# szlbiubiubiu/LAFS_CVPR2024

Measured on AMD Instinct MI355X. Metric: face-crops/sec/node (ViT-S LAFS pretrain, 2g+8l crops), higher is better.
Workload: dtype bf16; 1 GPU; vit_small/8 LAFS pretrain step, 2 global 112x112 + 8 local 48x48 crops, batch 64/GPU, out_dim 100000, drop_path 0.1, dp1; global_batch=64, parallelism=dp1, hip_graph=True, landmark_frontend_in_step=False, device_augmentation_in_step=False

## Files before the change

lafs_cvpr2024_amd/csrc/gemm_kres.hip:

```cpp
#include <stdlib.h>
#include "common.hpp"
#include "gemm_plan.hpp"
#include "ctx.hpp"

namespace {

typedef unsigned int u32x4_t __attribute__((ext_vector_type(4)));
typedef float f32x4v_t __attribute__((ext_vector_type(4)));

constexpr int KK = 384;
constexpr int CPR = KK / 8;
constexpr int ROWB = KK * 2;
constexpr int GROWS = 32;
constexpr int STAGE = GROWS * ROWB;
constexpr int NSTG = 3;
constexpr int NTH = 256;
constexpr int NDMA4 = STAGE / 16 / NTH;
constexpr int NKK = KK / 32;
constexpr int MAXN = 1536;
constexpr int FD = 8;
static_assert(CPR % 16 == 0 && STAGE % (16 * NTH) == 0, "stage layout");

struct KArgs {
  const bf16_t* A; const bf16_t* B;
  int M, N, lda, ldb;
  void* C; int ldc; void* C2; int ldc2;
  const float* bias; const float* resid; int ldr;
  const float* seq_scale; const int* row2seq;
  const bf16_t* aux; int ldaux;
  int cbn, items;
  int save_grad;
};

template <int N> __device__ __forceinline__ void wait_vm() { asm volatile("s_waitcnt vmcnt(%0)" ::"n"(N) : "memory"); }
__device__ __forceinline__ void fence() { asm volatile("" ::: "memory"); }
__device__ __forceinline__ void st16(void* p, unsigned a, unsigned b, unsigned c, unsigned d) {
  const u32x4_t v = {a, b, c, d};
  *reinterpret_cast<u32x4_t*>(p) = v;
}
__device__ __forceinline__ void st16f(void* p, float a, float b, float c, float d) {
  const f32x4v_t v = {a, b, c, d};
  *reinterpret_cast<f32x4v_t*>(p) = v;
}

template <int EPI, bool HAS_U> struct EpiOps {
  static constexpr bool F32 = (EPI == LAFS_EPI_RESID_F32);
  static constexpr int S = F32 ? 8 : ((EPI == LAFS_EPI_BF16_GELU && HAS_U) ? 8 : 4);
  static constexpr int P = F32 ? 8 : ((EPI == LAFS_EPI_DGELU_BF16) ? 4 : 0);
};

template <int EPI, bool HAS_U>
__global__ __launch_bounds__(NTH, 2) void gemm_kres_kernel(KArgs p) {
  constexpr int UROWS = 128, NDMA = NDMA4;
  constexpr int S = EpiOps<EPI, HAS_U>::S, P = EpiOps<EPI, HAS_U>::P;
  constexpr bool F32 = EpiOps<EPI, HAS_U>::F32;
  constexpr bool AUX_IS_GRAD = (EPI == LAFS_EPI_DGELU_BF16) && !HAS_U;
  __shared__ __attribute__((aligned(16))) unsigned char smem[NSTG * STAGE];
  __shared__ __attribute__((aligned(16))) float sbias[MAXN];
  const int tid = threadIdx.x, lane = tid & 63;
  const int wave = __builtin_amdgcn_readfirstlane(tid >> 6);
  const int t = lane & 15, q = lane >> 4;
  const int G = (int)gridDim.x, per = G >> 3;
  const int id = (blockIdx.x & 7) * per + (blockIdx.x >> 3);
  const int ib = (int)((long)p.items * id / G), ie = (int)((long)p.items * (id + 1) / G);
  if (ie <= ib) return;

  for (int i = tid; i < p.N; i += NTH) sbias[i] = p.bias ? p.bias[i] : 0.f;
  __syncthreads();

  int doff[NDMA];
#pragma unroll
  for (int i = 0; i < NDMA; ++i) {
    const int x = i * NTH + tid, rho = x / CPR, cp = x % CPR, c = cp ^ (rho & 15);
    const int s16 = rho & 15, gi = rho >> 4;
    const int rowrel = F32 ? rho : (8 * (s16 >> 2) + 4 * gi + (s16 & 3));
    doff[i] = (rowrel * p.ldb + c * 8) * 2;
  }
  const int cbn = p.cbn;
  const unsigned lds0 = lds_addr_of(smem);
  int pstage = 0;
  auto issue = [&](int k) {
    const int cb = (k >> 1) % cbn;
    const bf16_t* base = p.B + (size_t)(cb * 64 + 32 * (k & 1)) * p.ldb;
    const unsigned st = lds0 + pstage * STAGE + wave * 1024;
    pstage = (pstage + 1 == NSTG) ? 0 : pstage + 1;
    fence();
#pragma unroll
    for (int i = 0; i < NDMA; ++i) lds_dma16_m0_s(base, (unsigned)doff[i], st + i * (NTH * 16));
    fence();
  };
  auto issue_rows = [&](int mu, int w, int buf) {
    const unsigned st = lds0 + buf * STAGE + wave * 1024;
    fence();
#pragma unroll
    for (int i = 0; i < NDMA; ++i) {
      const int x = i * NTH + tid, rho = x / CPR, cp = x % CPR, c = cp ^ (rho & 15);
      const int row = min(mu * UROWS + w * 32 + rho, p.M - 1);
      lds_dma16_m0(p.A + (size_t)row * p.lda + c * 8, st + i * (NTH * 16));
    }
    fence();
  };

  int foff[4];
#pragma unroll
  for (int i = 0; i < 4; ++i) {
    foff[i] = t * ROWB + (((4 * i + q) ^ t) << 4);
    asm volatile("" : "+v"(foff[i]));
  }
  bf16x8_t areg[2][NKK];
  f32x4_t acc[2][2][2];
  uint4 pre[P > 0 ? P : 1];
  float sc[2] = {1.0f, 1.0f};
  int cur_mu = -1;
  bool active = false;
  int m0 = 0;

  auto fetch = [&](int item, uint4 (&dst)[P > 0 ? P : 1]) {
    if (P == 0) return;
    const int it = min(item, p.items - 1);
    const int mu = it / cbn, n0 = (it - mu * cbn) * 64;
#pragma unroll
    for (int i = 0; i < P; ++i) {
      const int b = i & 1, x = i >> 1;
      const int mr = min(mu * UROWS + wave * 32 + t + 16 * b, p.M - 1);
      if (F32) dst[i] = *reinterpret_cast<const uint4*>(p.resid + (size_t)mr * p.ldr + n0 + 16 * x + 4 * q);
      else dst[i] = *reinterpret_cast<const uint4*>(p.aux + (size_t)mr * p.ldaux + n0 + 32 * x + 8 * q);
    }
    fence();
  };
  auto bias_init = [&](f32x4_t (&a)[2][2], int n0, int g) {
#pragma unroll
    for (int gi = 0; gi < 2; ++gi) {
      const int n = F32 ? n0 + 16 * (2 * g + gi) + 4 * q : n0 + 32 * g + 8 * q + 4 * gi;
#pragma unroll
      for (int b = 0; b < 2; ++b) a[gi][b] = *reinterpret_cast<const f32x4_t*>(sbias + n);
    }
  };
  auto mfma_stage = [&](int stage, f32x4_t (&a)[2][2]) {
    __builtin_amdgcn_sched_barrier(0);
    const unsigned char* st = smem + stage * STAGE;
#pragma unroll
    for (int kk = 0; kk < NKK; ++kk)
#pragma unroll
      for (int gi = 0; gi < 2; ++gi) {
        const bf16x8_t w = *reinterpret_cast<const bf16x8_t*>(st + foff[kk & 3] + (kk >> 2) * 256 + gi * (16 * ROWB));
        a[gi][0] = mfma16(w, areg[0][kk], a[gi][0]);
        a[gi][1] = mfma16(w, areg[1][kk], a[gi][1]);
      }
    __builtin_amdgcn_sched_group_barrier(0x100, FD, 0);
#pragma unroll
    for (int i = 0; i < 2 * NKK - FD; ++i) {
      __builtin_amdgcn_sched_group_barrier(0x008, 2, 0);
      __builtin_amdgcn_sched_group_barrier(0x100, 1, 0);
    }
    __builtin_amdgcn_sched_group_barrier(0x008, 2 * FD, 0);
    __builtin_amdgcn_sched_barrier(0);
  };

  auto read_rows = [&](int buf) {
    const unsigned char* st = smem + buf * STAGE;
#pragma unroll
    for (int b = 0; b < 2; ++b)
#pragma unroll
      for (int kk = 0; kk < NKK; ++kk)
        areg[b][kk] = *reinterpret_cast<const bf16x8_t*>(st + foff[kk & 3] + (kk >> 2) * 256 + b * (16 * ROWB));
    asm volatile("s_waitcnt lgkmcnt(0)" ::: "memory");
  };
  int stage = 0;
  bool fresh = false;
  for (int it = ib; it < ie; ++it) {
    const int mu = it / cbn, cb = it - mu * cbn;
    const int k0 = 2 * it;
    const bool feed_next = (it + 1 < ie) && ((it + 1) / cbn == mu);
    bias_init(acc[0], cb * 64, 0);
    if (mu != cur_mu) {
      cur_mu = mu;
      m0 = mu * UROWS + wave * 32 + t;
      active = (mu * UROWS + wave * 32) < p.M;
      if (EPI == LAFS_EPI_RESID_F32 && p.seq_scale != nullptr) {
#pragma unroll
        for (int b = 0; b < 2; ++b) sc[b] = p.seq_scale[p.row2seq[min(m0 + 16 * b, p.M - 1)]];
      }
      wait_vm<0>();
      __builtin_amdgcn_s_barrier();
      issue_rows(mu, 0, 0); issue_rows(mu, 1, 1); issue_rows(mu, 2, 2);
      wait_vm<0>();
      __builtin_amdgcn_s_barrier();
      if (wave < 3) read_rows(wave);
      __builtin_amdgcn_s_barrier();
      issue_rows(mu, 3, 0);
      pstage = 1;
      issue(k0);
      issue(k0 + 1);
      wait_vm<2 * NDMA>();
      __builtin_amdgcn_s_barrier();
      if (wave == 3) read_rows(0);
      stage = 1;
      wait_vm<NDMA>();
      fresh = true;
    } else {
      if (active) wait_vm<NDMA + S + P>(); else wait_vm<NDMA + P>();
    }
    __builtin_amdgcn_s_barrier();
    if (feed_next) issue(k0 + 2);
    bias_init(acc[1], cb * 64, 1);
    mfma_stage(stage, acc[0]);
    stage = (stage + 1 == NSTG) ? 0 : stage + 1;
    if (fresh) {
      if (feed_next) wait_vm<NDMA>(); else wait_vm<0>();
    } else if (feed_next) {
      if (active) wait_vm<NDMA + S + P>(); else wait_vm<NDMA + P>();
    } else {
      if (active) wait_vm<S + P>(); else wait_vm<P>();
    }
    fresh = false;
    __builtin_amdgcn_s_barrier();
    if (feed_next) issue(k0 + 3);
    fetch(it, pre);
    mfma_stage(stage, acc[1]);
    stage = (stage + 1 == NSTG) ? 0 : stage + 1;

    fence();
    const int n0 = cb * 64;
    if (active) {
#pragma unroll
      for (int b = 0; b < 2; ++b) {
        const int m = m0 + 16 * b;
        const bool rowok = (m < p.M);
        if (F32) {
#pragma unroll
          for (int x = 0; x < 4; ++x) {
            const int g = x >> 1, gi = x & 1;
            const int n = n0 + 16 * x + 4 * q;
            const uint4 r4 = pre[x * 2 + b];
            float v0 = acc[g][gi][b][0], v1 = acc[g][gi][b][1], v2 = acc[g][gi][b][2], v3 = acc[g][gi][b][3];
            v0 = __uint_as_float(r4.x) + sc[b] * v0; v1 = __uint_as_float(r4.y) + sc[b] * v1;
            v2 = __uint_as_float(r4.z) + sc[b] * v2; v3 = __uint_as_float(r4.w) + sc[b] * v3;
            if (rowok) st16f(reinterpret_cast<float*>(p.C) + (size_t)m * p.ldc + n, v0, v1, v2, v3);
          }
        } else {
          float v[2][8];
#pragma unroll
          for (int g = 0; g < 2; ++g) {
            v[g][0] = acc[g][0][b][0]; v[g][1] = acc[g][0][b][1]; v[g][2] = acc[g][0][b][2]; v[g][3] = acc[g][0][b][3];
            v[g][4] = acc[g][1][b][0]; v[g][5] = acc[g][1][b][1]; v[g][6] = acc[g][1][b][2]; v[g][7] = acc[g][1][b][3];
            if (EPI == LAFS_EPI_DGELU_BF16) {
              const uint4 a4 = pre[g * 2 + b];
              if constexpr (AUX_IS_GRAD) {
                v[g][0] *= bf_lo(a4.x); v[g][1] *= bf_hi(a4.x); v[g][2] *= bf_lo(a4.y); v[g][3] *= bf_hi(a4.y);
                v[g][4] *= bf_lo(a4.z); v[g][5] *= bf_hi(a4.z); v[g][6] *= bf_lo(a4.w); v[g][7] *= bf_hi(a4.w);
              } else {
                v[g][0] *= gelu_grad_f(bf_lo(a4.x)); v[g][1] *= gelu_grad_f(bf_hi(a4.x)); v[g][2] *= gelu_grad_f(bf_lo(a4.y)); v[g][3] *= gelu_grad_f(bf_hi(a4.y));
                v[g][4] *= gelu_grad_f(bf_lo(a4.z)); v[g][5] *= gelu_grad_f(bf_hi(a4.z)); v[g][6] *= gelu_grad_f(bf_lo(a4.w)); v[g][7] *= gelu_grad_f(bf_hi(a4.w));
              }
            }
          }
          float dv[2][8];
          const bool both = (EPI == LAFS_EPI_BF16_GELU) && HAS_U && p.save_grad;
          if (both) {
#pragma unroll
            for (int g = 0; g < 2; ++g)
#pragma unroll
              for (int e = 0; e < 8; ++e) { float gv; gelu_both_f(v[g][e], gv, dv[g][e]); v[g][e] = gv; }
#pragma unroll
            for (int g = 0; g < 2; ++g) {
              const int n = n0 + 32 * g + 8 * q;
              if (rowok) st16(reinterpret_cast<bf16_t*>(p.C) + (size_t)m * p.ldc + n, pack_bf2(dv[g][0], dv[g][1]), pack_bf2(dv[g][2], dv[g][3]),
                              pack_bf2(dv[g][4], dv[g][5]), pack_bf2(dv[g][6], dv[g][7]));
            }
          }
          if ((EPI != LAFS_EPI_BF16_GELU || HAS_U) && !both) {
#pragma unroll
            for (int g = 0; g < 2; ++g) {
              const int n = n0 + 32 * g + 8 * q;
              if (rowok) st16(reinterpret_cast<bf16_t*>(p.C) + (size_t)m * p.ldc + n, pack_bf2(v[g][0], v[g][1]), pack_bf2(v[g][2], v[g][3]),
                              pack_bf2(v[g][4], v[g][5]), pack_bf2(v[g][6], v[g][7]));
            }
          }
          if (EPI == LAFS_EPI_BF16_GELU) {
            if (!both) {
#pragma unroll
              for (int g = 0; g < 2; ++g)
#pragma unroll
                for (int e = 0; e < 8; ++e) v[g][e] = gelu_f(v[g][e]);
            }
#pragma unroll
            for (int g = 0; g < 2; ++g) {
              const int n = n0 + 32 * g + 8 * q;
              if (rowok) st16(reinterpret_cast<bf16_t*>(p.C2) + (size_t)m * p.ldc2 + n, pack_bf2(v[g][0], v[g][1]), pack_bf2(v[g][2], v[g][3]),
                              pack_bf2(v[g][4], v[g][5]), pack_bf2(v[g][6], v[g][7]));
            }
          }
        }
      }
    }
    fence();
  }
}

template <int EPI, bool HAS_U>
int launch(const KArgs& a, int grid, hipStream_t s) {
  hipLaunchKernelGGL((gemm_kres_kernel<EPI, HAS_U>), dim3(grid), dim3(NTH), 0, s, a);
  LAFS_LAUNCH_CHECK();
  return LAFS_OK;
}

}

bool lafs_kres_eligible(const lafs_gemm_nt_args* g, NtPlan* p) {
  const int mask = lafs_ctx_opt(g->ctx, LAFS_OPT_KRES_MASK);
  const int e = g->epilogue;
  const int bit = e == LAFS_EPI_BF16 ? 1 : (e == LAFS_EPI_BF16_GELU ? 2 : (e == LAFS_EPI_RESID_F32 ? 4 : (e == LAFS_EPI_DGELU_BF16 ? 8 : 0)));
  if (!(mask & bit)) return false;
  if (g->splits > 1 || g->operand_f16) return false;
  if (g->K != KK || g->N % 64 != 0 || g->N > MAXN || g->N < 64 || g->M < 2048) return false;
  if (g->drop_p > 0.f) return false;
  if (g->C == nullptr && g->ldc % 8 != 0) return false;
  const int items = ((g->M + 127) / 128) * (g->N / 64);
  const int min_items = lafs_ctx_opt(g->ctx, LAFS_OPT_KRES_MIN_ITEMS);
  const int g_comm_cus = lafs_ctx_opt(g->ctx, LAFS_OPT_COMM_CUS);
  int grid = 512;
  while (grid > 8 && items / grid < min_items) grid >>= 1;
  if (g_comm_cus > 0 && grid > 2 * (256 - g_comm_cus)) grid = (2 * (256 - g_comm_cus)) & ~7;
  p->info = { 1,  128,  64,  KK,  NTH,  0,  1,  grid};
  return true;
}

int lafs_kres_launch(const lafs_gemm_nt_args* g, const NtPlan& p, hipStream_t stream) {
  const int e = g->epilogue;
  KArgs a;
  a.A = (const bf16_t*)g->A; a.B = (const bf16_t*)g->B; a.M = g->M; a.N = g->N; a.lda = g->lda; a.ldb = g->ldb;
  a.C = g->C; a.ldc = g->ldc; a.C2 = g->C2; a.ldc2 = g->ldc2;
  a.bias = (e == LAFS_EPI_DGELU_BF16) ? nullptr : g->bias;
  a.resid = g->resid; a.ldr = g->ldr; a.seq_scale = g->seq_scale; a.row2seq = g->row2seq;
  a.aux = (const bf16_t*)g->aux; a.ldaux = g->ldaux;
  a.cbn = g->N / 64;
  a.save_grad = (g->act == LAFS_GELU_SAVE_GRAD && (e == LAFS_EPI_BF16_GELU || e == LAFS_EPI_DGELU_BF16)) ? 1 : 0;
  a.items = ((g->M + 127) / 128) * a.cbn;
  const int grid = p.info.workgroups;
  switch (e) {
    case LAFS_EPI_BF16: return launch<LAFS_EPI_BF16, true>(a, grid, stream);
    case LAFS_EPI_BF16_GELU:
      return g->C != nullptr ? launch<LAFS_EPI_BF16_GELU, true>(a, grid, stream) : launch<LAFS_EPI_BF16_GELU, false>(a, grid, stream);
    case LAFS_EPI_RESID_F32: return launch<LAFS_EPI_RESID_F32, true>(a, grid, stream);
    default:
      return a.save_grad ? launch<LAFS_EPI_DGELU_BF16, false>(a, grid, stream) : launch<LAFS_EPI_DGELU_BF16, true>(a, grid, stream);
  }
}
```

lafs_cvpr2024_amd/csrc/gemm_plan.hpp:

```cpp
#pragma once
#include "lafs_hip.h"

struct NtPlan {
  lafs_gemm_nt_plan_info info;
  int inst, klen;
  int geo;
};

bool lafs_kres_eligible(const lafs_gemm_nt_args* g, NtPlan* p);
int lafs_kres_launch(const lafs_gemm_nt_args* g, const NtPlan& p, hipStream_t stream);
bool lafs_big_eligible(const lafs_gemm_nt_args* g, NtPlan* p);
int lafs_big_launch(const lafs_gemm_nt_args* g, const NtPlan& p, hipStream_t stream);
```

Baseline: 45550 face-crops/s.

## Partition K-resident GEMM work by row-unit aligned column splits

Replaces the flat linear split of (row-unit, column-block) items across workgroups with a partition where each workgroup owns one 128-row unit and a contiguous slice of its column blocks, when that balances well enough. The restructured loop nests column blocks inside row units, so each workgroup loads its A rows exactly once and avoids row reloads at item-range boundaries. Bias loading now overlaps with the initial row DMA, and the min-items grid-shrinking knob is dropped. This can change the grid size and load balance, and it falls back to the linear split when the partition would be too uneven.

```diff
diff --git a/lafs_cvpr2024_amd/csrc/gemm_kres.hip b/lafs_cvpr2024_amd/csrc/gemm_kres.hip
--- a/lafs_cvpr2024_amd/csrc/gemm_kres.hip
+++ b/lafs_cvpr2024_amd/csrc/gemm_kres.hip
@@ -28,9 +28,18 @@
   const float* bias; const float* resid; int ldr;
   const float* seq_scale; const int* row2seq;
   const bf16_t* aux; int ldaux;
-  int cbn, items;
+  int cbn, units, parts;
   int save_grad;
 };
+
+struct KresGrid { int parts, grid; };
+inline KresGrid kres_partition(int units, int cbn, int slots) {
+  int parts = slots / units;
+  parts = parts > cbn ? cbn : parts;
+  const long items = (long)units * cbn;
+  if (parts < 1 || 2L * ((cbn + parts - 1) / parts) * slots > 2 * items + 3L * slots) return {0, slots};
+  return {parts, (units * parts + 7) & ~7};
+}
 
 template <int N> __device__ __forceinline__ void wait_vm() { asm volatile("s_waitcnt vmcnt(%0)" ::"n"(N) : "memory"); }
 __device__ __forceinline__ void fence() { asm volatile("" ::: "memory"); }
@@ -62,11 +71,19 @@
   const int t = lane & 15, q = lane >> 4;
   const int G = (int)gridDim.x, per = G >> 3;
   const int id = (blockIdx.x & 7) * per + (blockIdx.x >> 3);
-  const int ib = (int)((long)p.items * id / G), ie = (int)((long)p.items * (id + 1) / G);
-  if (ie <= ib) return;
-
-  for (int i = tid; i < p.N; i += NTH) sbias[i] = p.bias ? p.bias[i] : 0.f;
-  __syncthreads();
+  const int cbn = p.cbn;
+  int ib, ie;
+  if (p.parts > 0) {
+    const int part = id % p.parts, unit = id / p.parts;
+    if (unit >= p.units) return;
+    ib = unit * cbn + cbn * part / p.parts;
+    ie = unit * cbn + cbn * (part + 1) / p.parts;
+  } else {
+    const long items = (long)p.units * cbn;
+    ib = (int)(items * id / G);
+    ie = (int)(items * (id + 1) / G);
+    if (ie <= ib) return;
+  }
 
   int doff[NDMA];
 #pragma unroll
@@ -76,12 +93,10 @@
     const int rowrel = F32 ? rho : (8 * (s16 >> 2) + 4 * gi + (s16 & 3));
     doff[i] = (rowrel * p.ldb + c * 8) * 2;
   }
-  const int cbn = p.cbn;
   const unsigned lds0 = lds_addr_of(smem);
   int pstage = 0;
   auto issue = [&](int k) {
-    const int cb = (k >> 1) % cbn;
-    const bf16_t* base = p.B + (size_t)(cb * 64 + 32 * (k & 1)) * p.ldb;
+    const bf16_t* base = p.B + (size_t)(32 * k) * p.ldb;
     const unsigned st = lds0 + pstage * STAGE + wave * 1024;
     pstage = (pstage + 1 == NSTG) ? 0 : pstage + 1;
     fence();
@@ -111,18 +126,16 @@
   f32x4_t acc[2][2][2];
   uint4 pre[P > 0 ? P : 1];
   float sc[2] = {1.0f, 1.0f};
-  int cur_mu = -1;
   bool active = false;
   int m0 = 0;
 
-  auto fetch = [&](int item, uint4 (&dst)[P > 0 ? P : 1]) {
+  auto fetch = [&](int cb, uint4 (&dst)[P > 0 ? P : 1]) {
     if (P == 0) return;
-    const int it = min(item, p.items - 1);
-    const int mu = it / cbn, n0 = (it - mu * cbn) * 64;
+    const int n0 = cb * 64;
 #pragma unroll
     for (int i = 0; i < P; ++i) {
       const int b = i & 1, x = i >> 1;
-      const int mr = min(mu * UROWS + wave * 32 + t + 16 * b, p.M - 1);
+      const int mr = min(m0 + 16 * b, p.M - 1);
       if (F32) dst[i] = *reinterpret_cast<const uint4*>(p.resid + (size_t)mr * p.ldr + n0 + 16 * x + 4 * q);
       else dst[i] = *reinterpret_cast<const uint4*>(p.aux + (size_t)mr * p.ldaux + n0 + 32 * x + 8 * q);
     }
@@ -166,135 +179,134 @@
         areg[b][kk] = *reinterpret_cast<const bf16x8_t*>(st + foff[kk & 3] + (kk >> 2) * 256 + b * (16 * ROWB));
     asm volatile("s_waitcnt lgkmcnt(0)" ::: "memory");
   };
-  int stage = 0;
-  bool fresh = false;
-  for (int it = ib; it < ie; ++it) {
-    const int mu = it / cbn, cb = it - mu * cbn;
-    const int k0 = 2 * it;
-    const bool feed_next = (it + 1 < ie) && ((it + 1) / cbn == mu);
-    bias_init(acc[0], cb * 64, 0);
-    if (mu != cur_mu) {
-      cur_mu = mu;
-      m0 = mu * UROWS + wave * 32 + t;
-      active = (mu * UROWS + wave * 32) < p.M;
-      if (EPI == LAFS_EPI_RESID_F32 && p.seq_scale != nullptr) {
-#pragma unroll
-        for (int b = 0; b < 2; ++b) sc[b] = p.seq_scale[p.row2seq[min(m0 + 16 * b, p.M - 1)]];
+  const int mu0 = ib / cbn;
+  for (int mu = mu0; mu * cbn < ie; ++mu) {
+    const bool first_unit = (mu == mu0);
+    const int cb0 = max(ib - mu * cbn, 0), cb1 = min(ie - mu * cbn, cbn);
+    m0 = mu * UROWS + wave * 32 + t;
+    active = (mu * UROWS + wave * 32) < p.M;
+    if (!first_unit) __builtin_amdgcn_s_barrier();
+    issue_rows(mu, 0, 0); issue_rows(mu, 1, 1); issue_rows(mu, 2, 2);
+    if (first_unit)
+      for (int i = tid; i < p.N; i += NTH) sbias[i] = p.bias ? p.bias[i] : 0.f;
+    if (EPI == LAFS_EPI_RESID_F32 && p.seq_scale != nullptr) {
+#pragma unroll
+      for (int b = 0; b < 2; ++b) sc[b] = p.seq_scale[p.row2seq[min(m0 + 16 * b, p.M - 1)]];
+    }
+    wait_vm<0>();
+    __syncthreads();
+    if (wave < 3) read_rows(wave);
+    __builtin_amdgcn_s_barrier();
+    issue_rows(mu, 3, 0);
+    pstage = 1;
+    issue(2 * cb0);
+    issue(2 * cb0 + 1);
+    wait_vm<2 * NDMA>();
+    __builtin_amdgcn_s_barrier();
+    if (wave == 3) read_rows(0);
+    int stage = 1;
+    for (int cb = cb0; cb < cb1; ++cb) {
+      const int k0 = 2 * cb;
+      const bool first = (cb == cb0);
+      const bool feed_next = (cb + 1 < cb1);
+      bias_init(acc[0], cb * 64, 0);
+      if (first) wait_vm<NDMA>();
+      else if (active) wait_vm<NDMA + S + P>();
+      else wait_vm<NDMA + P>();
+      __builtin_amdgcn_s_barrier();
+      if (feed_next) issue(k0 + 2);
+      bias_init(acc[1], cb * 64, 1);
+      mfma_stage(stage, acc[0]);
+      stage = (stage + 1 == NSTG) ? 0 : stage + 1;
+      if (first) {
+        if (feed_next) wait_vm<NDMA>(); else wait_vm<0>();
+      } else if (feed_next) {
+        if (active) wait_vm<NDMA + S + P>(); else wait_vm<NDMA + P>();
+      } else {
+        if (active) wait_vm<S + P>(); else wait_vm<P>();
       }
-      wait_vm<0>();
       __builtin_amdgcn_s_barrier();
-      issue_rows(mu, 0, 0); issue_rows(mu, 1, 1); issue_rows(mu, 2, 2);
-      wait_vm<0>();
-      __builtin_amdgcn_s_barrier();
-      if (wave < 3) read_rows(wave);
-      __builtin_amdgcn_s_barrier();
-      issue_rows(mu, 3, 0);
-      pstage = 1;
-      issue(k0);
-      issue(k0 + 1);
-      wait_vm<2 * NDMA>();
-      __builtin_amdgcn_s_barrier();
-      if (wave == 3) read_rows(0);
-      stage = 1;
-      wait_vm<NDMA>();
-      fresh = true;
-    } else {
-      if (active) wait_vm<NDMA + S + P>(); else wait_vm<NDMA + P>();
-    }
-    __builtin_amdgcn_s_barrier();
-    if (feed_next) issue(k0 + 2);
-    bias_init(acc[1], cb * 64, 1);
-    mfma_stage(stage, acc[0]);
-    stage = (stage + 1 == NSTG) ? 0 : stage + 1;
-    if (fresh) {
-      if (feed_next) wait_vm<NDMA>(); else wait_vm<0>();
-    } else if (feed_next) {
-      if (active) wait_vm<NDMA + S + P>(); else wait_vm<NDMA + P>();
-    } else {
-      if (active) wait_vm<S + P>(); else wait_vm<P>();
-    }
-    fresh = false;
-    __builtin_amdgcn_s_barrier();
-    if (feed_next) issue(k0 + 3);
-    fetch(it, pre);
-    mfma_stage(stage, acc[1]);
-    stage = (stage + 1 == NSTG) ? 0 : stage + 1;
-
-    fence();
-    const int n0 = cb * 64;
-    if (active) {
-#pragma unroll
-      for (int b = 0; b < 2; ++b) {
-        const int m = m0 + 16 * b;
-        const bool rowok = (m < p.M);
-        if (F32) {
-#pragma unroll
-          for (int x = 0; x < 4; ++x) {
-            const int g = x >> 1, gi = x & 1;
-            const int n = n0 + 16 * x + 4 * q;
-            const uint4 r4 = pre[x * 2 + b];
-            float v0 = acc[g][gi][b][0], v1 = acc[g][gi][b][1], v2 = acc[g][gi][b][2], v3 = acc[g][gi][b][3];
-            v0 = __uint_as_float(r4.x) + sc[b] * v0; v1 = __uint_as_float(r4.y) + sc[b] * v1;
-            v2 = __uint_as_float(r4.z) + sc[b] * v2; v3 = __uint_as_float(r4.w) + sc[b] * v3;
-            if (rowok) st16f(reinterpret_cast<float*>(p.C) + (size_t)m * p.ldc + n, v0, v1, v2, v3);
-          }
-        } else {
-          float v[2][8];
-#pragma unroll
-          for (int g = 0; g < 2; ++g) {
-            v[g][0] = acc[g][0][b][0]; v[g][1] = acc[g][0][b][1]; v[g][2] = acc[g][0][b][2]; v[g][3] = acc[g][0][b][3];
-            v[g][4] = acc[g][1][b][0]; v[g][5] = acc[g][1][b][1]; v[g][6] = acc[g][1][b][2]; v[g][7] = acc[g][1][b][3];
-            if (EPI == LAFS_EPI_DGELU_BF16) {
-              const uint4 a4 = pre[g * 2 + b];
-              if constexpr (AUX_IS_GRAD) {
-                v[g][0] *= bf_lo(a4.x); v[g][1] *= bf_hi(a4.x); v[g][2] *= bf_lo(a4.y); v[g][3] *= bf_hi(a4.y);
-                v[g][4] *= bf_lo(a4.z); v[g][5] *= bf_hi(a4.z); v[g][6] *= bf_lo(a4.w); v[g][7] *= bf_hi(a4.w);
-              } else {
-                v[g][0] *= gelu_grad_f(bf_lo(a4.x)); v[g][1] *= gelu_grad_f(bf_hi(a4.x)); v[g][2] *= gelu_grad_f(bf_lo(a4.y)); v[g][3] *= gelu_grad_f(bf_hi(a4.y));
-                v[g][4] *= gelu_grad_f(bf_lo(a4.z)); v[g][5] *= gelu_grad_f(bf_hi(a4.z)); v[g][6] *= gelu_grad_f(bf_lo(a4.w)); v[g][7] *= gelu_grad_f(bf_hi(a4.w));
-              }
-            }
-          }
-          float dv[2][8];
-          const bool both = (EPI == LAFS_EPI_BF16_GELU) && HAS_U && p.save_grad;
-          if (both) {
-#pragma unroll
-            for (int g = 0; g < 2; ++g)
-#pragma unroll
-              for (int e = 0; e < 8; ++e) { float gv; gelu_both_f(v[g][e], gv, dv[g][e]); v[g][e] = gv; }
+      if (feed_next) issue(k0 + 3);
+      fetch(cb, pre);
+      mfma_stage(stage, acc[1]);
+      stage = (stage + 1 == NSTG) ? 0 : stage + 1;
+
+      fence();
+      const int n0 = cb * 64;
+      if (active) {
+#pragma unroll
+        for (int b = 0; b < 2; ++b) {
+          const int m = m0 + 16 * b;
+          const bool rowok = (m < p.M);
+          if (F32) {
+#pragma unroll
+            for (int x = 0; x < 4; ++x) {
+              const int g = x >> 1, gi = x & 1;
+              const int n = n0 + 16 * x + 4 * q;
+              const uint4 r4 = pre[x * 2 + b];
+              float v0 = acc[g][gi][b][0], v1 = acc[g][gi][b][1], v2 = acc[g][gi][b][2], v3 = acc[g][gi][b][3];
+              v0 = __uint_as_float(r4.x) + sc[b] * v0; v1 = __uint_as_float(r4.y) + sc[b] * v1;
+              v2 = __uint_as_float(r4.z) + sc[b] * v2; v3 = __uint_as_float(r4.w) + sc[b] * v3;
+              if (rowok) st16f(reinterpret_cast<float*>(p.C) + (size_t)m * p.ldc + n, v0, v1, v2, v3);
+            }
+          } else {
+            float v[2][8];
 #pragma unroll
             for (int g = 0; g < 2; ++g) {
-              const int n = n0 + 32 * g + 8 * q;
-              if (rowok) st16(reinterpret_cast<bf16_t*>(p.C) + (size_t)m * p.ldc + n, pack_bf2(dv[g][0], dv[g][1]), pack_bf2(dv[g][2], dv[g][3]),
-                              pack_bf2(dv[g][4], dv[g][5]), pack_bf2(dv[g][6], dv[g][7]));
-            }
-          }
-          if ((EPI != LAFS_EPI_BF16_GELU || HAS_U) && !both) {
-#pragma unroll
-            for (int g = 0; g < 2; ++g) {
-              const int n = n0 + 32 * g + 8 * q;
-              if (rowok) st16(reinterpret_cast<bf16_t*>(p.C) + (size_t)m * p.ldc + n, pack_bf2(v[g][0], v[g][1]), pack_bf2(v[g][2], v[g][3]),
-                              pack_bf2(v[g][4], v[g][5]), pack_bf2(v[g][6], v[g][7]));
-            }
-          }
-          if (EPI == LAFS_EPI_BF16_GELU) {
-            if (!both) {
+              v[g][0] = acc[g][0][b][0]; v[g][1] = acc[g][0][b][1]; v[g][2] = acc[g][0][b][2]; v[g][3] = acc[g][0][b][3];
+              v[g][4] = acc[g][1][b][0]; v[g][5] = acc[g][1][b][1]; v[g][6] = acc[g][1][b][2]; v[g][7] = acc[g][1][b][3];
+              if (EPI == LAFS_EPI_DGELU_BF16) {
+                const uint4 a4 = pre[g * 2 + b];
+                if constexpr (AUX_IS_GRAD) {
+                  v[g][0] *= bf_lo(a4.x); v[g][1] *= bf_hi(a4.x); v[g][2] *= bf_lo(a4.y); v[g][3] *= bf_hi(a4.y);
+                  v[g][4] *= bf_lo(a4.z); v[g][5] *= bf_hi(a4.z); v[g][6] *= bf_lo(a4.w); v[g][7] *= bf_hi(a4.w);
+                } else {
+                  v[g][0] *= gelu_grad_f(bf_lo(a4.x)); v[g][1] *= gelu_grad_f(bf_hi(a4.x)); v[g][2] *= gelu_grad_f(bf_lo(a4.y)); v[g][3] *= gelu_grad_f(bf_hi(a4.y));
+                  v[g][4] *= gelu_grad_f(bf_lo(a4.z)); v[g][5] *= gelu_grad_f(bf_hi(a4.z)); v[g][6] *= gelu_grad_f(bf_lo(a4.w)); v[g][7] *= gelu_grad_f(bf_hi(a4.w));
+                }
+              }
+            }
+            float dv[2][8];
+            const bool both = (EPI == LAFS_EPI_BF16_GELU) && HAS_U && p.save_grad;
+            if (both) {
 #pragma unroll
               for (int g = 0; g < 2; ++g)
 #pragma unroll
-                for (int e = 0; e < 8; ++e) v[g][e] = gelu_f(v[g][e]);
-            }
-#pragma unroll
-            for (int g = 0; g < 2; ++g) {
-              const int n = n0 + 32 * g + 8 * q;
-              if (rowok) st16(reinterpret_cast<bf16_t*>(p.C2) + (size_t)m * p.ldc2 + n, pack_bf2(v[g][0], v[g][1]), pack_bf2(v[g][2], v[g][3]),
-                              pack_bf2(v[g][4], v[g][5]), pack_bf2(v[g][6], v[g][7]));
+                for (int e = 0; e < 8; ++e) { float gv; gelu_both_f(v[g][e], gv, dv[g][e]); v[g][e] = gv; }
+#pragma unroll
+              for (int g = 0; g < 2; ++g) {
+                const int n = n0 + 32 * g + 8 * q;
+                if (rowok) st16(reinterpret_cast<bf16_t*>(p.C) + (size_t)m * p.ldc + n, pack_bf2(dv[g][0], dv[g][1]), pack_bf2(dv[g][2], dv[g][3]),
+                                pack_bf2(dv[g][4], dv[g][5]), pack_bf2(dv[g][6], dv[g][7]));
+              }
+            }
+            if ((EPI != LAFS_EPI_BF16_GELU || HAS_U) && !both) {
+#pragma unroll
+              for (int g = 0; g < 2; ++g) {
+                const int n = n0 + 32 * g + 8 * q;
+                if (rowok) st16(reinterpret_cast<bf16_t*>(p.C) + (size_t)m * p.ldc + n, pack_bf2(v[g][0], v[g][1]), pack_bf2(v[g][2], v[g][3]),
+                                pack_bf2(v[g][4], v[g][5]), pack_bf2(v[g][6], v[g][7]));
+              }
+            }
+            if (EPI == LAFS_EPI_BF16_GELU) {
+              if (!both) {
+#pragma unroll
+                for (int g = 0; g < 2; ++g)
+#pragma unroll
+                  for (int e = 0; e < 8; ++e) v[g][e] = gelu_f(v[g][e]);
+              }
+#pragma unroll
+              for (int g = 0; g < 2; ++g) {
+                const int n = n0 + 32 * g + 8 * q;
+                if (rowok) st16(reinterpret_cast<bf16_t*>(p.C2) + (size_t)m * p.ldc2 + n, pack_bf2(v[g][0], v[g][1]), pack_bf2(v[g][2], v[g][3]),
+                                pack_bf2(v[g][4], v[g][5]), pack_bf2(v[g][6], v[g][7]));
+              }
             }
           }
         }
       }
-    }
-    fence();
+      fence();
+    }
   }
 }
 
@@ -316,13 +328,12 @@
   if (g->K != KK || g->N % 64 != 0 || g->N > MAXN || g->N < 64 || g->M < 2048) return false;
   if (g->drop_p > 0.f) return false;
   if (g->C == nullptr && g->ldc % 8 != 0) return false;
-  const int items = ((g->M + 127) / 128) * (g->N / 64);
-  const int min_items = lafs_ctx_opt(g->ctx, LAFS_OPT_KRES_MIN_ITEMS);
   const int g_comm_cus = lafs_ctx_opt(g->ctx, LAFS_OPT_COMM_CUS);
-  int grid = 512;
-  while (grid > 8 && items / grid < min_items) grid >>= 1;
-  if (g_comm_cus > 0 && grid > 2 * (256 - g_comm_cus)) grid = (2 * (256 - g_comm_cus)) & ~7;
-  p->info = { 1,  128,  64,  KK,  NTH,  0,  1,  grid};
+  int slots = 512;
+  if (g_comm_cus > 0 && slots > 2 * (256 - g_comm_cus)) slots = (2 * (256 - g_comm_cus)) & ~7;
+  const KresGrid kg = kres_partition((g->M + 127) / 128, g->N / 64, slots);
+  p->info = { 1,  128,  64,  KK,  NTH,  0,  1,  kg.grid};
+  p->kres_parts = kg.parts;
   return true;
 }
 
@@ -336,7 +347,8 @@
   a.aux = (const bf16_t*)g->aux; a.ldaux = g->ldaux;
   a.cbn = g->N / 64;
   a.save_grad = (g->act == LAFS_GELU_SAVE_GRAD && (e == LAFS_EPI_BF16_GELU || e == LAFS_EPI_DGELU_BF16)) ? 1 : 0;
-  a.items = ((g->M + 127) / 128) * a.cbn;
+  a.units = (g->M + 127) / 128;
+  a.parts = p.kres_parts;
   const int grid = p.info.workgroups;
   switch (e) {
     case LAFS_EPI_BF16: return launch<LAFS_EPI_BF16, true>(a, grid, stream);
diff --git a/lafs_cvpr2024_amd/csrc/gemm_plan.hpp b/lafs_cvpr2024_amd/csrc/gemm_plan.hpp
--- a/lafs_cvpr2024_amd/csrc/gemm_plan.hpp
+++ b/lafs_cvpr2024_amd/csrc/gemm_plan.hpp
@@ -5,6 +5,7 @@
   lafs_gemm_nt_plan_info info;
   int inst, klen;
   int geo;
+  int kres_parts;
 };
 
 bool lafs_kres_eligible(const lafs_gemm_nt_args* g, NtPlan* p);
```

Measured after the change: 46120 face-crops/s (median of 6 runs). No clear change (+1.3%).
